# tkwa/iit

Measured on AMD Instinct MI355X. Metric: IIT (base,source) intervened pairs/sec, IOI GPT-2-small, IOI_ModelPair IIT+strict+behavior step, higher is better.
Workload: dtype bf16; 1 GPU; model=gpt2-small 12L/768d/12H (TL GPT-2 cfg, LNPre, gelu_new, V=50257), global_batch=256, seq_len=16, parallelism=dp1, engine=native, graphs=True

## Files before the change

csrc/gemm_dual.hip:

```cpp
#include "gemm_glds_body.h"

namespace {

template <int BM_, int BN_, int NS_, int NW_ = 4, int OCC_ = 2>
struct Cfg {
  static constexpr int BM = BM_, BN = BN_, NS = NS_, NW = NW_, OCC = OCC_;
  static constexpr int SMEM = GldsSmem<BM_, BN_, NS_, NW_, 64, OCC_>::BYTES;
};

struct Prefetch {
  const char* p[2];
  long bytes[2];
  int wgs;
};

__device__ __forceinline__ void prefetch_part(const Prefetch& pf, int part) {
  unsigned acc = 0u;
#pragma unroll
  for (int r = 0; r < 2; ++r) {
    if (!pf.p[r] || pf.bytes[r] <= 0) continue;
    const long gran = (pf.bytes[r] + 63) / 64;
    const long per = (gran + pf.wgs - 1) / pf.wgs;
    const long g0 = (long)part * per;
    const long g1 = g0 + per < gran ? g0 + per : gran;
    const char* base = pf.p[r];
    for (long g = g0 + threadIdx.x; g < g1; g += (long)blockDim.x * 8) {
      unsigned v[8];
#pragma unroll
      for (int u = 0; u < 8; ++u) {
        const long gg = g + (long)u * blockDim.x;
        v[u] = gg < g1 ? *(const unsigned*)(base + gg * 64) : 0u;
      }
#pragma unroll
      for (int u = 0; u < 8; ++u) acc ^= v[u];
    }
  }
  asm volatile("" ::"v"(acc));
}

template <class TW, int EW, class TX, int EX>
__global__ __launch_bounds__(TW::NW * 64, TW::OCC) void gemm_dual_kernel(G2Args pw, G2Args px, int w_tiles,
                                                                         int w_splits, int x_tiles, Prefetch pf) {
  static_assert(TW::NW == TX::NW && TW::OCC == TX::OCC, "one launch geometry");
  __shared__ __attribute__((aligned(16))) char smem[TW::SMEM > TX::SMEM ? TW::SMEM : TX::SMEM];
  if ((int)blockIdx.x < pf.wgs) {
    prefetch_part(pf, blockIdx.x);
    return;
  }
  const int b = blockIdx.x - pf.wgs;
  const int nw = w_tiles * w_splits;
  if (b < nw) {
    gemm_glds_body<TW::BM, TW::BN, TW::NS, true, true, EW, TW::NW, 64, TW::OCC>(pw, b % w_tiles, w_tiles,
                                                                                b / w_tiles, w_splits, smem);
// ... 135 lines not shown
```

csrc/layer_norm.hip:

```cpp
#include "common.h"
#include <initializer_list>
#include <stdlib.h>
#include <type_traits>

template <int W>
struct Pack;

template <>
struct Pack<4> {
  float4 v;
  static __device__ __forceinline__ Pack splat(float s) { return {make_float4(s, s, s, s)}; }
  static __device__ __forceinline__ Pack load(const float* p, long i) { return {((const float4*)p)[i]}; }
  static __device__ __forceinline__ Pack load(const __bf16* p, long i) {
    const bf16x4 t = ((const bf16x4*)p)[i];
    return {make_float4(bf2f(t[0]), bf2f(t[1]), bf2f(t[2]), bf2f(t[3]))};
  }
  template <class F, class... P>
  static __device__ __forceinline__ Pack map(F f, const P&... a) {
    return {make_float4(f(a.v.x...), f(a.v.y...), f(a.v.z...), f(a.v.w...))};
  }
  __device__ __forceinline__ float hsum() const { return (v.x + v.y) + (v.z + v.w); }
  template <int PIN>
  static __device__ __forceinline__ float dot(const Pack& a, const Pack& b) {
    if constexpr (PIN == 1)
// ... 41 lines not shown

struct RowSel {
  unsigned long long mask;
  int S;
  int Tb;
};

__device__ __forceinline__ bool sel_hit(const RowSel& sel, int row) {
  return sel.mask != 0ull && row < sel.Tb && ((sel.mask >> (row % sel.S)) & 1ull);
}

template <int W, int N>
__global__ __launch_bounds__(256) void ln_fwd_kernel(const float* __restrict__ x, const float* __restrict__ w,
                                                     const float* __restrict__ b, __bf16* __restrict__ y,
                                                     float* __restrict__ mean_out, float* __restrict__ rstd_out,
                                                     int T, int d, float eps, RowSel sel, float* __restrict__ y32) {
  using P = Pack<W>;
  const int row = blockIdx.x * 4 + (threadIdx.x >> 6);
  const int lane = threadIdx.x & 63;
  if (row >= T) return;
  const int dn = d / W;
  const long xat = (long)(sel_hit(sel, row) ? row + sel.Tb : row) * dn, yat = (long)row * dn;
  P v[N];
  float s = 0.f;
#pragma unroll
  for (int i = 0; i < N; ++i) {
    const int c = lane + i * 64;
    v[i] = c < dn ? P::load(x, xat + c) : P::splat(0.f);
    s += v[i].hsum();
  }
  const float mu = wave_sum(s) / d;
  float s2 = 0.f;
#pragma unroll
// ... 300 lines not shown
    if (n <= 1) f(W, ln_int<1>{}); else if (n <= 2) f(W, ln_int<2>{}); else if (n <= 3) f(W, ln_int<3>{});
    else if (n <= 4) f(W, ln_int<4>{}); else if (n <= 6) f(W, ln_int<6>{}); else if (n <= 8) f(W, ln_int<8>{});
    else if (n <= 12) f(W, ln_int<12>{}); else f(W, ln_int<16>{});
  } else {
    const ln_int<1> W;
    if (n <= 4) f(W, ln_int<4>{}); else if (n <= 16) f(W, ln_int<16>{}); else if (n <= 32) f(W, ln_int<32>{});
    else f(W, ln_int<64>{});
  }
}

template <class F>
static void ln_flag(bool b, F&& f) {
  if (b) f(std::true_type{}); else f(std::false_type{});
}

IIT_EXPORT int iit_ln_fwd(const float* x, const float* w, const float* b, void* y, float* y32, float* mean,
                          float* rstd, int T, int d, float eps, unsigned long long pos_mask, int S, int Tb,
                          void* stream) {
  if (pos_mask && (S <= 0 || S > 64 || 2 * (long)Tb > T)) return (int)hipErrorInvalidValue;
  const bool vec = ln_vec(d, {f32_rows(x), bf16_rows(y), f32_rows(y32), f32_rows(w), f32_rows(b)});
  if (d > 4096 || (y32 && !vec)) return (int)hipErrorInvalidValue;
  const RowSel sel{pos_mask, S > 0 ? S : 1, Tb};
  ln_dispatch(vec, d, [&](auto W, auto N) {
    hipLaunchKernelGGL((ln_fwd_kernel<W, N>), dim3((T + 3) / 4), dim3(256), 0, (hipStream_t)stream, x, w, b,
                       (__bf16*)y, mean, rstd, T, d, eps, sel, y32);
  });
  return hipGetLastError();
}

IIT_EXPORT int iit_ln_bwd_part_rows() { return 4 * ln_part_r(); }

IIT_EXPORT int iit_ln_bwd(const void* dy, int dy_f32, const void* x, int x_is_xhat16, const float* mean,
                          const float* rstd, const float* w, float* dx, const float* dres, void* dx16, float* dw,
                          float* db, float* part, const float* dy2, int T, int d, int accumulate,
                          unsigned long long pos_mask, int S, void* stream) {
  if (d > 4096 || (pos_mask && (S <= 0 || S > 64))) return (int)hipErrorInvalidValue;
  const LnPtr dyp = dy_f32 ? f32_rows(dy) : bf16_rows(dy), xp = x_is_xhat16 ? bf16_rows(x) : f32_rows(x);
  const bool vec = ln_vec(d, {dyp, xp, f32_rows(dx), f32_rows(dres), f32_rows(w), bf16_rows(dx16)});
  const bool fused = vec && !x_is_xhat16 && part && dw && db && d <= 1024 &&
                     ln_vec(d, {f32_rows(dw), f32_rows(db), f32_rows(part), f32_rows(dy2)});
  if ((dy2 && !fused) || (x_is_xhat16 && (!vec || w || dw || db))) return (int)hipErrorInvalidValue;
  const RowSel sel{pos_mask, S > 0 ? S : 1, T};
// ... 55 lines not shown
```

iit_amd/models/transformer.py:

```python
from __future__ import annotations

import math
import os
from typing import List, Optional, Union

import torch
from torch import nn

from ..engine.plan import RunPlan, Splice, scale_site as _scale_site, zero_grad_site as _zero_grad_site
from ..hooks.hook_points import HookedRootModule, HookPoint
from ..ops import select_ops
from ..ops.torch_ops import TorchOps
from .config import HookedTransformerConfig, make_config


def _hip_ops():
    from ..ops import hip_ops
    return hip_ops


def _flash_ok(q: torch.Tensor) -> bool:
    return q.is_cuda and q.dtype == torch.bfloat16 and _hip_ops().flash_supported(q)


# ... 70 lines not shown
        self.eps = cfg.eps
        self.rms = rms
        self.w = nn.Parameter(torch.ones(cfg.d_model)) if affine else None
        self.b = nn.Parameter(torch.zeros(cfg.d_model)) if (affine and not rms) else None
        self.hook_scale = HookPoint()
        self.hook_normalized = HookPoint()

    @staticmethod
    def make(cfg: HookedTransformerConfig, kind: Optional[str]) -> Optional["LayerNormSite"]:
        if kind is None:
            return None
        if kind not in ("LN", "LNPre", "RMS", "RMSPre"):
            raise NotImplementedError(f"normalization_type {kind}")
        return LayerNormSite(cfg, affine=kind in ("LN", "RMS"), rms=kind in ("RMS", "RMSPre"))

    def run(self, x, run: _Run, twin: bool = False):
        live = run.live(self.hook_scale) or run.live(self.hook_normalized)
        if self.rms:
            hs = (lambda t: run.site(self.hook_scale, t)) if live else None
            hn = (lambda t: run.site(self.hook_normalized, t)) if live else None
            return TorchOps.rms_norm(run.ops, x, self.w, self.eps, hook_scale=hs, hook_normalized=hn)
        if live or not run.ops.fused:
            return TorchOps.layer_norm(
                run.ops, x, self.w, self.b, self.eps,
                hook_scale=lambda t: run.site(self.hook_scale, t),
                hook_normalized=lambda t: run.site(self.hook_normalized, t),
            )
        if twin and self.w is not None and hasattr(run.ops, "layer_norm_twin"):
            return run.ops.layer_norm_twin(x, self.w, self.b, self.eps)
        return run.ops.layer_norm(x, self.w, self.b, self.eps)


def rotary_tables(cfg: HookedTransformerConfig):
    rd = cfg.rotary_dim or cfg.d_head
    pos = torch.arange(cfg.n_ctx, dtype=torch.float64)
    freq = cfg.rotary_base ** (-torch.arange(0, rd, 2, dtype=torch.float64) / rd)
    ang = pos[:, None] * freq[None, :]
    ang = ang.repeat_interleave(2, dim=-1) if cfg.rotary_adjacent_pairs else torch.cat([ang, ang], dim=-1)
    return ang.sin().float(), ang.cos().float()


class Attention(nn.Module):
    def __init__(self, cfg: HookedTransformerConfig, layer: int):
        super().__init__()
        H, d, dh = cfg.n_heads, cfg.d_model, cfg.d_head
# ... 149 lines not shown
        self.attn = Attention(cfg, layer)
        if not cfg.attn_only:
            self.mlp = MLP(cfg)
        self.hook_attn_in = HookPoint()
        self.hook_q_input = HookPoint()
        self.hook_k_input = HookPoint()
        self.hook_v_input = HookPoint()
        self.hook_mlp_in = HookPoint()
        self.hook_attn_out = HookPoint()
        self.hook_mlp_out = HookPoint()
        self.hook_resid_pre = HookPoint()
        if not cfg.attn_only:
            self.hook_resid_mid = HookPoint()
        self.hook_resid_post = HookPoint()

    def _norm(self, ln, x, run):
        if ln is None:
            return x.to(run.ops.dtype)
        return ln.run(x, run)

    def _norm_fork(self, ln, x, run):
        if ln is None or run.live(ln.hook_scale) or run.live(ln.hook_normalized) or not x.requires_grad:
            return self._norm(ln, x, run), x
        if ln.rms:
            fork = getattr(run.ops, "rms_norm_fork", None)
            out = fork(x, ln.w, ln.eps) if fork is not None else None
            return out if out is not None else (self._norm(ln, x, run), x)
        fork = getattr(run.ops, "layer_norm_fork", None)
        if fork is None:
            return self._norm(ln, x, run), x
        return fork(x, ln.w, ln.b, ln.eps)

    def last_position_ok(self, run: _Run) -> bool:
        if self.cfg.use_attn_result:
            return False
        sites = [self.hook_attn_out, self.hook_resid_post, self.hook_mlp_out]
        if not self.cfg.attn_only:
            sites += [self.hook_resid_mid, self.hook_mlp_in, self.mlp.hook_pre, self.mlp.hook_post]
            if self.mlp.gated:
                sites.append(self.mlp.hook_pre_linear)
            if self.ln2 is not None:
                sites += [self.ln2.hook_scale, self.ln2.hook_normalized]
        return not any(run.live(h) for h in sites)

    def forward(self, resid: torch.Tensor, run: _Run, last_only: bool = False) -> torch.Tensor:
        ops = run.ops
        attn = self.attn
        resid = run.site(self.hook_resid_pre, resid)

        spl = run.whole_splice(attn.hook_z.name)
        ln1_live = self.ln1 is not None and (run.live(self.ln1.hook_scale) or run.live(self.ln1.hook_normalized))
        if spl is not None and not attn.inner_live(run) and not ln1_live:
            z = run.site(attn.hook_z, spl.src.to(ops.dtype), spliced=True)
        else:
            x, resid = self._norm_fork(self.ln1, resid, run)
            z, spliced = attn.compute_z(x, run)
            z = run.site(attn.hook_z, z, spliced=spliced)
        if last_only:
            z, resid = z[:, -1:].contiguous(), resid[:, -1:].contiguous()
        attn_out_live = run.live(self.hook_attn_out) or self.cfg.use_attn_result
        if self.cfg.use_attn_result:
            result = run.site(attn.hook_result, ops.o_result(z, attn.W_O))
            attn_out = result.sum(-2) + ops.w(attn.b_O)
            attn_out = run.site(self.hook_attn_out, attn_out)
            resid_mid_pre = ops.residual(resid, attn_out)
        elif attn_out_live or not (ops.fused or getattr(ops, "fuses_residual", False)):
            attn_out = run.site(self.hook_attn_out, ops.o_proj(z, attn.W_O, attn.b_O))
            resid_mid_pre = ops.residual(resid, attn_out)
        else:
            resid_mid_pre = ops.o_proj_residual(z, attn.W_O, attn.b_O, resid)

        if self.cfg.attn_only:
            return run.site(self.hook_resid_post, resid_mid_pre)
        resid_mid = run.site(self.hook_resid_mid, resid_mid_pre)

        mlp = self.mlp
        spl = run.whole_splice(mlp.hook_post.name)
        ln2_live = self.ln2 is not None and (run.live(self.ln2.hook_scale) or run.live(self.ln2.hook_normalized))
        pre_lin_live = mlp.gated and run.live(mlp.hook_pre_linear)
        if spl is not None and not run.live(mlp.hook_pre) and not ln2_live and not pre_lin_live:
            post = run.site(mlp.hook_post, spl.src.to(ops.dtype), spliced=True)
        elif (not mlp.gated and getattr(ops, "mlp_gelu_residual", None) is not None
              and self.cfg.act_fn in ("gelu_new", "gelu_fast", "gelu_pytorch_tanh")
              and not (ln2_live or run.live(mlp.hook_pre) or run.live(mlp.hook_post) or run.live(self.hook_mlp_out))):
            x, resid_mid = self._norm_fork(self.ln2, resid_mid, run)
            resid_post = ops.mlp_gelu_residual(x, mlp.W_in, mlp.b_in, mlp.W_out, mlp.b_out, resid_mid)
            return run.site(self.hook_resid_post, resid_post)
        else:
            x, resid_mid = self._norm_fork(self.ln2, resid_mid, run)
            pre_hook = (lambda t: run.site(mlp.hook_pre, t)) if run.live(mlp.hook_pre) else None
            spliced = False
            if mlp.gated:
                lin_hook = (lambda t: run.site(mlp.hook_pre_linear, t)) if run.live(mlp.hook_pre_linear) else None
                pspl = run.plan.splice.get(mlp.hook_post.name) if run.plan is not None else None
                if pspl and len(pspl) == 1 and not pspl[0].whole and pre_hook is None and lin_hook is None:
                    _, post, spliced = TorchOps.mlp_gated_in(ops, x, mlp.W_gate, mlp.W_in, mlp.b_in,
                                                             self.cfg.act_fn, splice=pspl[0])
                else:
                    _, post = TorchOps.mlp_gated_in(ops, x, mlp.W_gate, mlp.W_in, mlp.b_in, self.cfg.act_fn,
                                                    hook_pre=pre_hook, hook_pre_linear=lin_hook)
            else:
                _, post = ops.mlp_in(x, mlp.W_in, mlp.b_in, self.cfg.act_fn, hook_pre=pre_hook)
            post = run.site(mlp.hook_post, post, spliced=spliced)
        if run.live(self.hook_mlp_out) or not (ops.fused or getattr(ops, "fuses_residual", False)):
# ... 10 lines not shown
            return False
        if self.ln1 is None or self.ln1.rms or (not cfg.attn_only and (self.ln2 is None or self.ln2.rms)):
            return False
        if not cfg.attn_only and (self.mlp.gated or cfg.act_fn not in ("gelu_new", "gelu_fast", "gelu_pytorch_tanh")):
            return False
        return True

    def forward_paired(self, p, run: _Run, sites, stop_after: str, captures, last_only: bool = False):
        ops = run.ops
        attn = self.attn
        zname = attn.hook_z.name
        zs = sites.get(zname)
        causal = self.cfg.attention_dir == "causal"
        S, H, dh = p.full.shape[1], self.cfg.n_heads, self.cfg.d_head
        mirror = ops.pair_heads_ok(S, dh) and H <= 64
        if zs is not None and any(ix.is_everything() for ix in zs):
            with torch.no_grad():
                x = ops.layer_norm(p.src, self.ln1.w, self.ln1.b, self.ln1.eps)
                q, k, v = ops.qkv(x, attn.W_Q, attn.W_K, attn.W_V, attn.b_Q, attn.b_K, attn.b_V)
                if mirror:
                    zf = ops.attention_dual(q, causal, attn.attn_scale)
                else:
                    z_src = ops.attention(q, k, v, causal, attn.attn_scale)
                    zf = torch.cat([z_src, z_src])
            z = _hip_ops().Paired(zf[:p.nb], zf)
            resid = p
        else:
            x, resid = ops.pair_layer_norm_fork(p, self.ln1.w, self.ln1.b, self.ln1.eps)
            qkv = ops.pair_qkv(x, attn.W_Q, attn.W_K, attn.W_V, attn.b_Q, attn.b_K, attn.b_V)
            heads, rest = None, list(zs or ())
            z = None
            if mirror and len(rest) == 1:
                heads = Splice(rest[0], None).head_mask(H)
                if heads is not None:
                    rest = []
                else:
                    z = ops.pair_attention_spliced(qkv, causal, attn.attn_scale, rest[0])
                    if z is not None:
                        rest = []
            if z is None:
                z = ops.pair_attention(qkv, causal, attn.attn_scale, heads=heads)
            for ix in rest:
                z = ops.pair_splice(z, ix)
        if zs is not None:
            captures[zname] = z.src
        if zname == stop_after:
            return self._finish_after_attn(z.base, resid.base, run, last_only), False
        resid_mid = ops.pair_o_proj_residual(z, attn.W_O, attn.b_O, resid)
        if self.cfg.attn_only:
            return resid_mid, True
        mlp = self.mlp
        pname = mlp.hook_post.name
        ps = sites.get(pname)
        erf = False
        if ps is None:
            x, resid2 = ops.pair_layer_norm_fork(resid_mid, self.ln2.w, self.ln2.b, self.ln2.eps)
            return ops.pair_mlp_gelu_residual(x, mlp.W_in, mlp.b_in, mlp.W_out, mlp.b_out, resid2, erf=erf), True
        if any(ix.is_everything() for ix in ps):
            with torch.no_grad():
                x = ops.layer_norm(resid_mid.src, self.ln2.w, self.ln2.b, self.ln2.eps)
                _, post_src = ops.mlp_in(x, mlp.W_in, mlp.b_in, self.cfg.act_fn)
            qf = torch.cat([post_src, post_src])
            post = _hip_ops().Paired(qf[:post_src.shape[0]], qf)
            resid2 = resid_mid
        else:
            x, resid2 = ops.pair_layer_norm_fork(resid_mid, self.ln2.w, self.ln2.b, self.ln2.eps)
            done = ops.pair_mlp_in(x, mlp.W_in, mlp.b_in, erf=erf, index=ps[0]) if len(ps) == 1 else None
            if done is not None:
                _, post = done
            else:
                _, post = ops.pair_mlp_in(x, mlp.W_in, mlp.b_in, erf=erf)
                for ix in ps:
                    post = ops.pair_splice(post, ix)
        captures[pname] = post.src
        if pname == stop_after:
            return ops.mlp_out_residual(post.base, mlp.W_out, mlp.b_out, resid2.base), False
        return ops.pair_mlp_out_residual(post, mlp.W_out, mlp.b_out, resid2), True

    def paired_torch_ok(self, ops) -> bool:
        cfg = self.cfg
        if getattr(ops, "fused", True) or ops.dtype != torch.bfloat16 or cfg.use_attn_result:
# ... 64 lines not shown
            return resid_mid
        mlp = self.mlp
        x = self.ln2.run(resid_mid, run)
        _, post = TorchOps.mlp_gated_in(ops, x, mlp.W_gate, mlp.W_in, mlp.b_in, self.cfg.act_fn)
        return ops.residual(resid_mid, ops.mlp_out(post, mlp.W_out, mlp.b_out))

    def _finish_after_attn(self, z, resid, run: _Run, last_only: bool):
        ops = run.ops
        attn = self.attn
        if last_only:
            z, resid = z[:, -1:].contiguous(), resid[:, -1:].contiguous()
        resid_mid = ops.o_proj_residual(z, attn.W_O, attn.b_O, resid)
        if self.cfg.attn_only:
            return resid_mid
        mlp = self.mlp
        x, resid_mid = self._norm_fork(self.ln2, resid_mid, run)
        return ops.mlp_gelu_residual(x, mlp.W_in, mlp.b_in, mlp.W_out, mlp.b_out, resid_mid)


def qkv_arena_groups(blocks, cfg):
    H, d, dh = cfg.n_heads, cfg.d_model, cfg.d_head
    groups = []
    for blk in blocks:
        a = blk.attn
        Hkv = a.n_kv
        Wq = a.W_Q
        Wk, Wv = (a._W_K, a._W_V) if a.gqa else (a.W_K, a.W_V)
        bq = a.b_Q
        bk, bv = (a._b_K, a._b_V) if a.gqa else (a.b_K, a.b_V)
        if Wq.shape != (H, d, dh) or Wk.shape != (Hkv, d, dh) or Wv.shape != (Hkv, d, dh):
            continue
# ... 346 lines not shown
```

iit_amd/ops/build.py:

```python
from __future__ import annotations

import hashlib
import os
import subprocess
import sys

ROOT = os.path.dirname(os.path.dirname(os.path.dirname(os.path.abspath(__file__))))
CSRC = os.path.join(ROOT, "csrc")
OUT_DIR = os.path.join(ROOT, "iit_amd", "_native")
LIB = os.path.join(OUT_DIR, "libiit_hip.so")
OBJ_CACHE = os.path.join(ROOT, "build", "objcache")
SOURCES = ["gemm.hip", "gemm_glds.hip", "gemm_edge.hip", "gemm_dual.hip", "gemm_8ph.hip", "gemm_4w.hip", "conv_nhwc.hip", "kernels.hip", "layer_norm.hip", "attn_mfma.hip", "flash_attn.hip", "llama_ops.hip",
           "splice.hip", "ioi_hl.hip", "bn_nhwc.hip", "gemm_f32.hip", "attn_fp32.hip"]
EXTRA_FLAGS = {"gemm_glds.hip": ["-mllvm", "-amdgpu-mfma-vgpr-form"], "gemm_edge.hip": ["-mllvm", "-amdgpu-mfma-vgpr-form"], "conv_nhwc.hip": ["-mllvm", "-amdgpu-mfma-vgpr-form"], "gemm_dual.hip": ["-mllvm", "-amdgpu-mfma-vgpr-form"],
               "gemm_8ph.hip": ["-mllvm", "-amdgpu-mfma-vgpr-form"]}
HEADERS = ["common.h", "gemm_glds_body.h", "gemm_w4.h", "splice_spec.h"]
ARCH = os.environ.get("IIT_OFFLOAD_ARCH", "gfx950")


def _hipcc() -> str:
    for c in (os.environ.get("HIPCC"), "/opt/rocm/bin/hipcc"):
        if c and os.path.exists(c):
            return c
    return "hipcc"


def sources():
    return [os.path.join(CSRC, s) for s in SOURCES if os.path.exists(os.path.join(CSRC, s))]


def source_hash() -> str:
# ... 63 lines not shown
```

iit_amd/ops/hip_kernels.py:

```python
from __future__ import annotations

import ctypes
import math
import os
from typing import Optional, Sequence

import numpy as np
import torch

from . import build as _build

c_void_p, c_long, c_int, c_float, c_ull = ctypes.c_void_p, ctypes.c_long, ctypes.c_int, ctypes.c_float, ctypes.c_ulonglong

EPI_BF16, EPI_BF16_BIAS3, EPI_F32_RESID, EPI_GELU, EPI_DGELU, EPI_F32_ACC, EPI_F32_ACC_QKV, EPI_F32_STORE = range(8)
EPI_GELU_ERF = 8
EPI_DGELU_ERF = 9
MODE_NN, MODE_AKM, MODE_BKM, MODE_AF32, MODE_BF32 = 0, 1, 2, 4, 8

_LIB = None
GEMM_GROUP_M = 4
GEMM_DUAL_GROUP_M = 2

_SIGS = {
    "iit_gemm": [c_void_p] * 10 + [c_long] * 5 + [c_int] * 12 + [c_void_p],
    "iit_gemm_f32": [c_void_p] * 6 + [c_long] * 4 + [c_int] * 7 + [c_void_p],
    "iit_gemm_f32_ok": [c_void_p] * 6 + [c_long] * 4 + [c_int] * 7,
    "iit_attn_f32_lds": [c_int] * 3,
    "iit_attn_f32_waves": [c_int] * 3,
    "iit_attn_f32_ok": [c_void_p] * 4 + [c_int] * 4,
    "iit_attn_f32_fwd": [c_void_p] * 6 + [c_int] * 4 + [c_float, c_int, c_void_p],
    "iit_attn_f32_bwd": [c_void_p] * 9 + [c_int] * 4 + [c_float, c_int, c_void_p],
    "iit_gemm_glds": [c_void_p] * 8 + [c_long] * 5 + [c_int] * 8 + [c_void_p] * 4,
    "iit_gemm_glds_ok": [c_void_p] * 5 + [c_long] * 5 + [c_int] * 9,
    "iit_gemm_glds_sm": [c_void_p] * 8 + [c_long] * 5 + [c_int] * 8 + [c_void_p] * 3 + [c_int] + [c_void_p] * 3,
    "iit_embed_pos_fwd": [c_void_p, c_void_p, c_void_p, c_void_p, c_int, c_int, c_int, c_void_p],
    "iit_embed_pos_bwd": [c_void_p, c_void_p, c_void_p, c_void_p, c_int, c_int, c_int, c_void_p],
    "iit_ln_fwd": [c_void_p] * 7 + [c_int, c_int, c_float, c_ull, c_int, c_int, c_void_p],
    "iit_ln_bwd": [c_void_p, c_int, c_void_p, c_int] + [c_void_p] * 10 + [c_int, c_int, c_int, c_ull, c_int, c_void_p],
    "iit_ln_bwd_part_rows": [],
    "iit_attn_small_fwd": [c_void_p] * 4 + [c_ull, c_int, c_int, c_int, c_int, c_long, c_long, c_long, c_float, c_int,
                                            c_void_p],
    "iit_attn_small_bwd": [c_void_p] * 4 + [c_ull, c_int, c_int, c_int, c_int, c_long, c_long, c_float, c_int, c_void_p],
    "iit_attn_mfma_fwd": [c_void_p] * 4 + [c_ull, c_int, c_int, c_int, c_int, c_long, c_long, c_long, c_float, c_int,
                                           c_void_p],
    "iit_attn_mfma_fwd_pair": [c_void_p] * 4 + [c_ull, c_int, c_int, c_int, c_int, c_long, c_long, c_long, c_float,
                                                c_int, c_void_p, c_int, c_ull, c_void_p],
    "iit_attn_mfma_bwd": [c_void_p] * 4 + [c_ull, c_int, c_int, c_int, c_int, c_long, c_long, c_float, c_int, c_void_p],
    "iit_attn_mfma_fwd_spec": [c_void_p] * 3 + [c_int] * 4 + [c_long, c_long, c_float, c_int, c_int, c_void_p,
                                                               c_void_p],
    "iit_attn_mfma_bwd_spec": [c_void_p] * 4 + [c_int] * 4 + [c_long, c_long, c_float, c_int, c_void_p, c_void_p],
    "iit_ce_fwd": [c_void_p, c_long, c_void_p, c_void_p, c_void_p, c_void_p, c_int, c_int, c_void_p],
    "iit_ce_bwd": [c_void_p, c_long, c_void_p, c_void_p, c_void_p, c_float, c_void_p, c_long, c_int, c_int, c_int,
# ... 466 lines not shown
def splice(act, src, out, n, spec_ptr, f32, mode, scale=1.0):
    if CHECK_BOUNDS:
        _bounds("iit_splice", ("act", act, 1, n, n), ("out", out, 1, n, n))
    _check(lib().iit_splice(_p(act), _p(src), _p(out), n, spec_ptr, int(f32), int(mode), float(scale), _stream()),
           "iit_splice")


def embed_pos_fwd(tokens, W_E, W_pos, out, B, S, d):
    _check(lib().iit_embed_pos_fwd(_p(tokens), _p(W_E), _p(W_pos), _p(out), B * S, S, d, _stream()), "embed_pos_fwd")


def embed_pos_bwd(tokens, g, dWE, dWpos, B, S, d):
    _check(lib().iit_embed_pos_bwd(_p(tokens), _p(g), _p(dWE), _p(dWpos), B, S, d, _stream()), "embed_pos_bwd")


def _ln_fwd(what, x, w, b, y, y32, mean, rstd, T, d, eps, pos_mask=0, S=1, Tb=0) -> int:
    if CHECK_BOUNDS:
        _bounds(what, ("x", x, T, d, d), ("y", y, T, d, d), ("y32", y32, T, d, d), ("mean", mean, 1, T, T),
                ("rstd", rstd, 1, T, T))
    return lib().iit_ln_fwd(_p(x), _p(w), _p(b), _p(y), _p(y32), _p(mean), _p(rstd), T, d, eps, pos_mask, S, Tb, _stream())


def ln_fwd(x, w, b, y, mean, rstd, T, d, eps):
    _check(_ln_fwd("ln_fwd", x, w, b, y, None, mean, rstd, T, d, eps), "ln_fwd")


def ln_fwd_twin(x, w, b, y, y32, mean, rstd, T, d, eps) -> bool:
    return _ln_fwd("ln_fwd_twin", x, w, b, y, y32, mean, rstd, T, d, eps) == 0


def ln_fwd_sel(x, w, b, y, mean, rstd, T, d, eps, pos_mask: int, S: int, Tb: int):
    _check(_ln_fwd("ln_fwd_sel", x, w, b, y, None, mean, rstd, T, d, eps, pos_mask, S, Tb), "ln_fwd_sel")


_LN_PART_ROWS = [0]


def _ln_part(dw, T: int, d: int):
    if dw is None or os.environ.get("IIT_LN_FUSED_DWDB", "1") == "0":
        return None
    rows = _LN_PART_ROWS[0] or lib().iit_ln_bwd_part_rows()
    _LN_PART_ROWS[0] = rows
    return torch.empty(((T + rows - 1) // rows) * 2 * d, dtype=torch.float32, device=dw.device)


def _ln_bwd(what, dy, x, mean, rstd, w, dx, dw, db, T, d, *, accumulate=False, dres=None, dx16=None, dy2=None,
            pos_mask=0, S=1, xh16=False):
# ... 518 lines not shown
```

iit_amd/ops/hip_ops.py:

```python
from __future__ import annotations

import math
import os
from typing import Optional, Sequence

import torch
from torch.autograd import Function

from ..engine import grad_hooks
from . import hip_kernels as K
from .gemm_dispatch import gemm, gemm_pair
from .torch_ops import TorchOps, act_fn

BF16 = torch.bfloat16
F32 = torch.float32


def _pad8(n: int) -> int:
    return (n + 7) // 8 * 8


def _grad_slot(p: Optional[torch.Tensor]) -> Optional[torch.Tensor]:
    if p is None or not p.requires_grad:
        return None
# ... 310 lines not shown
        ctx.params = (W_E, W_pos)
        return out

    @staticmethod
    def backward(ctx, g):
        if g is None:
            return None, None, None
        (tok,) = ctx.saved_tensors
        W_E, W_pos = ctx.params
        B, S = tok.shape
        K.embed_pos_bwd(tok, g.contiguous(), _grad_slot(W_E), _grad_slot(W_pos), B, S, W_E.shape[1])
        _done(W_E, W_pos)
        return None, None, None


def _xhat16(w, b, d: int) -> bool:
    return w is None and b is None and d % 4 == 0 and d <= 4096 and os.environ.get("IIT_LN_XHAT16", "1") == "1"


def _ln_forward(ctx, x, w, b, eps, x_full=None, twin=False, xhat16=False, pos_mask=0):
    ctx.set_materialize_grads(False)
    rows = x if x_full is None else x_full
    lead, d = rows.shape[:-1], rows.shape[-1]
    x2 = _flat2(rows.float().contiguous())
    T2 = x2.shape[0]
    T = T2 * x.shape[0] // rows.shape[0]
    S = x.shape[1] if x.dim() == 3 else 1
    if xhat16:
        yf = torch.empty(T2, d, dtype=BF16, device=x.device)
        y = yf.view(*lead, d)
    else:
        y = torch.empty(*lead, d, dtype=BF16, device=x.device)
        yf = y.view(T2, d)
    y32 = torch.empty(*lead, d, dtype=F32, device=x.device) if twin else None
    mean = torch.empty(T2, dtype=F32, device=x.device)
    rstd = torch.empty(T2, dtype=F32, device=x.device)
    if pos_mask:
        K.ln_fwd_sel(x2, w, b, yf, mean, rstd, T2, d, eps, pos_mask, S, T)
    elif not twin or not K.ln_fwd_twin(x2, w, b, yf, y32.view(T2, d), mean, rstd, T2, d, eps):
        K.ln_fwd(x2, w, b, yf, mean, rstd, T2, d, eps)
        if twin:
            y32.copy_(y)
    ctx.save_for_backward((yf if xhat16 else x2)[:T], mean[:T], rstd[:T])
    ctx.params = (w, b)
    ctx.in_dtype = x.dtype
    ctx.sel = (pos_mask, S)
    return y, y32


def _ln_backward(ctx, dy, dres=None, dy2=None, sel=None):
    if dy is None and dy2 is not None:
        dy, dy2 = dy2.float(), None
    if dy is None:
        return dres
    xs, mean, rstd = ctx.saved_tensors
# ... 964 lines not shown
    box = []
    out = fn.apply(*args, box)
    return out, box[0]


class HipOps(TorchOps):
    name = "hip"
    fused = True

    def __init__(self, model):
        super().__init__(BF16)
        self.model = model
        self.shadow = ModelShadow(model)
        pol = os.environ.get("IIT_DUAL_PREFETCH", "auto")
        self.prefetch = pol == "1" or (pol == "auto" and type(model).__name__ != "HookedEncoder")
        self._layer_of = {}
        for i, blk in enumerate(model.blocks):
            self._layer_of[id(blk.attn.W_Q)] = i
            self._layer_of[id(blk.attn.W_O)] = i
            if not model.cfg.attn_only:
                self._layer_of[id(blk.mlp.W_in)] = i
                self._layer_of[id(blk.mlp.W_out)] = i

    def begin_forward(self):
        self.shadow.ensure()
        _PF_SEQ.clear()
        _PF_ON[0] = self.prefetch

    def _L(self, p):
        return self.shadow.layers[self._layer_of[id(p)]]

    def embed(self, tokens, W_E):
        return W_E[tokens]

    def pos_embed(self, batch, seq, W_pos, offset: int = 0):
        return W_pos[offset:offset + seq].unsqueeze(0).expand(batch, seq, W_pos.shape[-1])

    def embed_pos(self, tokens, W_E, W_pos):
        return EmbedPosFn.apply(tokens, W_E, W_pos)

    def residual(self, a, b):
        return a.float() + b.float()

    def w(self, p: torch.Tensor) -> torch.Tensor:
        return p.to(BF16)

    def layer_norm(self, x, w, b, eps):
        return LayerNormFn.apply(x, w, b, eps)

    def layer_norm_twin(self, x, w, b, eps):
        if os.environ.get("IIT_LN_TWIN", "1") == "0":
            return LayerNormFn.apply(x, w, b, eps)
        y, y32 = LayerNormTwinFn.apply(x, w, b, eps)
        y._iit_f32 = (y.data_ptr(), y._version, y32)
        return y

    def layer_norm_fork(self, x, w, b, eps):
        return LayerNormForkFn.apply(x, w, b, eps)

    def qkv(self, x, W_Q, W_K, W_V, b_Q, b_K, b_V):
        i = self._layer_of[id(W_Q)]
        packed = QKVFn.apply(x, self.shadow.layers[i], self.shadow.biases[i], W_Q, W_K, W_V, b_Q, b_K, b_V)
        q, k, v = packed[:, :, 0], packed[:, :, 1], packed[:, :, 2]
        q._iit_packed = k._iit_packed = v._iit_packed = packed
        return q, k, v

    def attention(self, q, k, v, causal, attn_scale, patch_heads: Optional[Sequence[int]] = None, patch_src=None,
                  hook_scores=None, hook_pattern=None, ignore=float("-inf")):
        S, dh = q.shape[1], q.shape[-1]
        if S > 16 and flash_supported(q):
            packed = getattr(q, "_iit_packed", None)
            if packed is not None and getattr(k, "_iit_packed", None) is packed and \
                    getattr(v, "_iit_packed", None) is packed and packed.is_contiguous():
# ... 88 lines not shown
                best_v, best_i = v, i
            else:
                upd = v > best_v
                best_v = torch.where(upd, v, best_v)
                best_i = torch.where(upd, i, best_i)
        return best_i.view(*lead)


    supports_pairs = True

    def pair_embed_pos(self, tokens, src_tokens, W_E, W_pos) -> Paired:
        full_tok = torch.cat([tokens, src_tokens]).contiguous()
        out, full = _one(EmbedPosPairFn, tokens, W_E, W_pos, full_tok)
        return Paired(out, full)

    def pair_layer_norm_fork(self, p: Paired, w, b, eps):
        box = []
        y, x_pass = LayerNormForkPairFn.apply(p.base, w, b, eps, p.full.float().contiguous(), box)
        return Paired(y, box[0]), Paired(x_pass, p.full)

    def pair_layer_norm(self, p: Paired, w, b, eps, pos_mask: int = 0, twin: bool = False) -> Paired:
        box = []
        if twin and not pos_mask and w is not None and os.environ.get("IIT_LN_TWIN", "1") != "0":
            y, y32 = LayerNormPairTwinFn.apply(p.base, w, b, eps, p.full.float().contiguous(), box)
            yf, yf32 = box[0]
            y._iit_f32 = (y.data_ptr(), y._version, y32)
            return Paired(y, yf, (y32, yf32))
        y = LayerNormPairFn.apply(p.base, w, b, eps, p.full.float().contiguous(), box, int(pos_mask))
        return Paired(y, box[0])

    @staticmethod
    def position_mask(index, shape) -> int:
        if len(shape) != 3 or shape[1] > 64:
            return 0
        ranges = index.to_ranges(tuple(shape))
        if ranges is None or ranges[0] != [(0, shape[0])] or ranges[2] != [(0, shape[2])]:
            return 0
        m = 0
        for lo, hi in ranges[1]:
            for s_ in range(lo, hi):
                m |= 1 << s_
        return m

# ... 116 lines not shown
```

Measured before the change: 16830 pairs/s.

## Prefetch next-layer GEMM weights into L2 from extra layer-norm workgroups

Adds extra workgroups to the layer-norm forward kernel. They touch the bf16 weights of the following GEMMs (QKV/O, MLP in/out) so those weights are pulled into cache before the GEMM runs. The prefetch helper moves into a shared header and is threaded through the LN forward paths, including pair and fork variants, gated by IIT_FWD_PREFETCH (auto enables it for HookedTransformer). The aim is to hide weight-load latency in the small-batch GEMMs, at the cost of extra LN launch work and cache pressure.

```diff
diff --git a/csrc/gemm_dual.hip b/csrc/gemm_dual.hip
--- a/csrc/gemm_dual.hip
+++ b/csrc/gemm_dual.hip
@@ -1,4 +1,5 @@
 #include "gemm_glds_body.h"
+#include "prefetch.h"
 
 namespace {
 
@@ -8,35 +9,6 @@
   static constexpr int SMEM = GldsSmem<BM_, BN_, NS_, NW_, 64, OCC_>::BYTES;
 };
 
-struct Prefetch {
-  const char* p[2];
-  long bytes[2];
-  int wgs;
-};
-
-__device__ __forceinline__ void prefetch_part(const Prefetch& pf, int part) {
-  unsigned acc = 0u;
-#pragma unroll
-  for (int r = 0; r < 2; ++r) {
-    if (!pf.p[r] || pf.bytes[r] <= 0) continue;
-    const long gran = (pf.bytes[r] + 63) / 64;
-    const long per = (gran + pf.wgs - 1) / pf.wgs;
-    const long g0 = (long)part * per;
-    const long g1 = g0 + per < gran ? g0 + per : gran;
-    const char* base = pf.p[r];
-    for (long g = g0 + threadIdx.x; g < g1; g += (long)blockDim.x * 8) {
-      unsigned v[8];
-#pragma unroll
-      for (int u = 0; u < 8; ++u) {
-        const long gg = g + (long)u * blockDim.x;
-        v[u] = gg < g1 ? *(const unsigned*)(base + gg * 64) : 0u;
-      }
-#pragma unroll
-      for (int u = 0; u < 8; ++u) acc ^= v[u];
-    }
-  }
-  asm volatile("" ::"v"(acc));
-}
 
 template <class TW, int EW, class TX, int EX>
 __global__ __launch_bounds__(TW::NW * 64, TW::OCC) void gemm_dual_kernel(G2Args pw, G2Args px, int w_tiles,
diff --git a/csrc/layer_norm.hip b/csrc/layer_norm.hip
--- a/csrc/layer_norm.hip
+++ b/csrc/layer_norm.hip
@@ -1,4 +1,5 @@
 #include "common.h"
+#include "prefetch.h"
 #include <initializer_list>
 #include <stdlib.h>
 #include <type_traits>
@@ -79,9 +80,14 @@
 __global__ __launch_bounds__(256) void ln_fwd_kernel(const float* __restrict__ x, const float* __restrict__ w,
                                                      const float* __restrict__ b, __bf16* __restrict__ y,
                                                      float* __restrict__ mean_out, float* __restrict__ rstd_out,
-                                                     int T, int d, float eps, RowSel sel, float* __restrict__ y32) {
+                                                     int T, int d, float eps, RowSel sel, float* __restrict__ y32,
+                                                     Prefetch pf) {
   using P = Pack<W>;
-  const int row = blockIdx.x * 4 + (threadIdx.x >> 6);
+  if ((int)blockIdx.x < pf.wgs) {
+    prefetch_part(pf, blockIdx.x);
+    return;
+  }
+  const int row = (blockIdx.x - pf.wgs) * 4 + (threadIdx.x >> 6);
   const int lane = threadIdx.x & 63;
   if (row >= T) return;
   const int dn = d / W;
@@ -412,18 +418,28 @@
   if (b) f(std::true_type{}); else f(std::false_type{});
 }
 
-IIT_EXPORT int iit_ln_fwd(const float* x, const float* w, const float* b, void* y, float* y32, float* mean,
-                          float* rstd, int T, int d, float eps, unsigned long long pos_mask, int S, int Tb,
-                          void* stream) {
+IIT_EXPORT int iit_ln_fwd_pf(const float* x, const float* w, const float* b, void* y, float* y32, float* mean,
+                             float* rstd, int T, int d, float eps, unsigned long long pos_mask, int S, int Tb,
+                             const void* pf0, long pf0_bytes, const void* pf1, long pf1_bytes, int pf_wgs,
+                             void* stream) {
   if (pos_mask && (S <= 0 || S > 64 || 2 * (long)Tb > T)) return (int)hipErrorInvalidValue;
   const bool vec = ln_vec(d, {f32_rows(x), bf16_rows(y), f32_rows(y32), f32_rows(w), f32_rows(b)});
   if (d > 4096 || (y32 && !vec)) return (int)hipErrorInvalidValue;
   const RowSel sel{pos_mask, S > 0 ? S : 1, Tb};
+  Prefetch pf{{(const char*)pf0, (const char*)pf1}, {pf0 ? pf0_bytes & ~3L : 0, pf1 ? pf1_bytes & ~3L : 0}, 0};
+  if (((uintptr_t)pf0 | (uintptr_t)pf1) & 3) return (int)hipErrorInvalidValue;
+  if ((pf.bytes[0] > 0 || pf.bytes[1] > 0) && pf_wgs > 0) pf.wgs = pf_wgs < 1024 ? pf_wgs : 1024;
   ln_dispatch(vec, d, [&](auto W, auto N) {
-    hipLaunchKernelGGL((ln_fwd_kernel<W, N>), dim3((T + 3) / 4), dim3(256), 0, (hipStream_t)stream, x, w, b,
-                       (__bf16*)y, mean, rstd, T, d, eps, sel, y32);
+    hipLaunchKernelGGL((ln_fwd_kernel<W, N>), dim3(pf.wgs + (T + 3) / 4), dim3(256), 0, (hipStream_t)stream, x, w, b,
+                       (__bf16*)y, mean, rstd, T, d, eps, sel, y32, pf);
   });
   return hipGetLastError();
+}
+
+IIT_EXPORT int iit_ln_fwd(const float* x, const float* w, const float* b, void* y, float* y32, float* mean,
+                          float* rstd, int T, int d, float eps, unsigned long long pos_mask, int S, int Tb,
+                          void* stream) {
+  return iit_ln_fwd_pf(x, w, b, y, y32, mean, rstd, T, d, eps, pos_mask, S, Tb, nullptr, 0, nullptr, 0, 0, stream);
 }
 
 IIT_EXPORT int iit_ln_bwd_part_rows() { return 4 * ln_part_r(); }
diff --git a/csrc/prefetch.h b/csrc/prefetch.h
--- /dev/null
+++ b/csrc/prefetch.h
@@ -0,0 +1,31 @@
+#pragma once
+
+struct Prefetch {
+  const char* p[2];
+  long bytes[2];
+  int wgs;
+};
+
+__device__ __forceinline__ void prefetch_part(const Prefetch& pf, int part) {
+  unsigned acc = 0u;
+#pragma unroll
+  for (int r = 0; r < 2; ++r) {
+    if (!pf.p[r] || pf.bytes[r] <= 0) continue;
+    const long gran = (pf.bytes[r] + 63) / 64;
+    const long per = (gran + pf.wgs - 1) / pf.wgs;
+    const long g0 = (long)part * per;
+    const long g1 = g0 + per < gran ? g0 + per : gran;
+    const char* base = pf.p[r];
+    for (long g = g0 + threadIdx.x; g < g1; g += (long)blockDim.x * 8) {
+      unsigned v[8];
+#pragma unroll
+      for (int u = 0; u < 8; ++u) {
+        const long gg = g + (long)u * blockDim.x;
+        v[u] = gg < g1 ? *(const unsigned*)(base + gg * 64) : 0u;
+      }
+#pragma unroll
+      for (int u = 0; u < 8; ++u) acc ^= v[u];
+    }
+  }
+  asm volatile("" ::"v"(acc));
+}
diff --git a/iit_amd/models/transformer.py b/iit_amd/models/transformer.py
--- a/iit_amd/models/transformer.py
+++ b/iit_amd/models/transformer.py
@@ -108,7 +108,7 @@
             raise NotImplementedError(f"normalization_type {kind}")
         return LayerNormSite(cfg, affine=kind in ("LN", "RMS"), rms=kind in ("RMS", "RMSPre"))
 
-    def run(self, x, run: _Run, twin: bool = False):
+    def run(self, x, run: _Run, twin: bool = False, prefetch=None):
         live = run.live(self.hook_scale) or run.live(self.hook_normalized)
         if self.rms:
             hs = (lambda t: run.site(self.hook_scale, t)) if live else None
@@ -120,9 +120,10 @@
                 hook_scale=lambda t: run.site(self.hook_scale, t),
                 hook_normalized=lambda t: run.site(self.hook_normalized, t),
             )
+        kw = {} if prefetch is None else {"prefetch": prefetch}
         if twin and self.w is not None and hasattr(run.ops, "layer_norm_twin"):
-            return run.ops.layer_norm_twin(x, self.w, self.b, self.eps)
-        return run.ops.layer_norm(x, self.w, self.b, self.eps)
+            return run.ops.layer_norm_twin(x, self.w, self.b, self.eps, **kw)
+        return run.ops.layer_norm(x, self.w, self.b, self.eps, **kw)
 
 
 def rotary_tables(cfg: HookedTransformerConfig):
@@ -302,14 +303,19 @@
             self.hook_resid_mid = HookPoint()
         self.hook_resid_post = HookPoint()
 
-    def _norm(self, ln, x, run):
+    @staticmethod
+    def _fwd_prefetch(ops, *Ws):
+        f = getattr(ops, "fwd_prefetch", None)
+        return f(*Ws) if f is not None else None
+
+    def _norm(self, ln, x, run, prefetch=None):
         if ln is None:
             return x.to(run.ops.dtype)
-        return ln.run(x, run)
-
-    def _norm_fork(self, ln, x, run):
+        return ln.run(x, run, prefetch=prefetch)
+
+    def _norm_fork(self, ln, x, run, prefetch=None):
         if ln is None or run.live(ln.hook_scale) or run.live(ln.hook_normalized) or not x.requires_grad:
-            return self._norm(ln, x, run), x
+            return self._norm(ln, x, run, prefetch), x
         if ln.rms:
             fork = getattr(run.ops, "rms_norm_fork", None)
             out = fork(x, ln.w, ln.eps) if fork is not None else None
@@ -317,7 +323,7 @@
         fork = getattr(run.ops, "layer_norm_fork", None)
         if fork is None:
             return self._norm(ln, x, run), x
-        return fork(x, ln.w, ln.b, ln.eps)
+        return fork(x, ln.w, ln.b, ln.eps, **({} if prefetch is None else {"prefetch": prefetch}))
 
     def last_position_ok(self, run: _Run) -> bool:
         if self.cfg.use_attn_result:
@@ -341,7 +347,7 @@
         if spl is not None and not attn.inner_live(run) and not ln1_live:
             z = run.site(attn.hook_z, spl.src.to(ops.dtype), spliced=True)
         else:
-            x, resid = self._norm_fork(self.ln1, resid, run)
+            x, resid = self._norm_fork(self.ln1, resid, run, self._fwd_prefetch(ops, attn.W_Q, attn.W_O))
             z, spliced = attn.compute_z(x, run)
             z = run.site(attn.hook_z, z, spliced=spliced)
         if last_only:
@@ -371,11 +377,11 @@
         elif (not mlp.gated and getattr(ops, "mlp_gelu_residual", None) is not None
               and self.cfg.act_fn in ("gelu_new", "gelu_fast", "gelu_pytorch_tanh")
               and not (ln2_live or run.live(mlp.hook_pre) or run.live(mlp.hook_post) or run.live(self.hook_mlp_out))):
-            x, resid_mid = self._norm_fork(self.ln2, resid_mid, run)
+            x, resid_mid = self._norm_fork(self.ln2, resid_mid, run, self._fwd_prefetch(ops, mlp.W_in, mlp.W_out))
             resid_post = ops.mlp_gelu_residual(x, mlp.W_in, mlp.b_in, mlp.W_out, mlp.b_out, resid_mid)
             return run.site(self.hook_resid_post, resid_post)
         else:
-            x, resid_mid = self._norm_fork(self.ln2, resid_mid, run)
+            x, resid_mid = self._norm_fork(self.ln2, resid_mid, run, self._fwd_prefetch(ops, mlp.W_in, mlp.W_out))
             pre_hook = (lambda t: run.site(mlp.hook_pre, t)) if run.live(mlp.hook_pre) else None
             spliced = False
             if mlp.gated:
@@ -416,9 +422,10 @@
         causal = self.cfg.attention_dir == "causal"
         S, H, dh = p.full.shape[1], self.cfg.n_heads, self.cfg.d_head
         mirror = ops.pair_heads_ok(S, dh) and H <= 64
+        pf1 = ops.fwd_prefetch(attn.W_Q, attn.W_O)
         if zs is not None and any(ix.is_everything() for ix in zs):
             with torch.no_grad():
-                x = ops.layer_norm(p.src, self.ln1.w, self.ln1.b, self.ln1.eps)
+                x = ops.layer_norm(p.src, self.ln1.w, self.ln1.b, self.ln1.eps, prefetch=pf1)
                 q, k, v = ops.qkv(x, attn.W_Q, attn.W_K, attn.W_V, attn.b_Q, attn.b_K, attn.b_V)
                 if mirror:
                     zf = ops.attention_dual(q, causal, attn.attn_scale)
@@ -428,7 +435,7 @@
             z = _hip_ops().Paired(zf[:p.nb], zf)
             resid = p
         else:
-            x, resid = ops.pair_layer_norm_fork(p, self.ln1.w, self.ln1.b, self.ln1.eps)
+            x, resid = ops.pair_layer_norm_fork(p, self.ln1.w, self.ln1.b, self.ln1.eps, prefetch=pf1)
             qkv = ops.pair_qkv(x, attn.W_Q, attn.W_K, attn.W_V, attn.b_Q, attn.b_K, attn.b_V)
             heads, rest = None, list(zs or ())
             z = None
@@ -455,18 +462,19 @@
         pname = mlp.hook_post.name
         ps = sites.get(pname)
         erf = False
+        pf2 = ops.fwd_prefetch(mlp.W_in, mlp.W_out)
         if ps is None:
-            x, resid2 = ops.pair_layer_norm_fork(resid_mid, self.ln2.w, self.ln2.b, self.ln2.eps)
+            x, resid2 = ops.pair_layer_norm_fork(resid_mid, self.ln2.w, self.ln2.b, self.ln2.eps, prefetch=pf2)
             return ops.pair_mlp_gelu_residual(x, mlp.W_in, mlp.b_in, mlp.W_out, mlp.b_out, resid2, erf=erf), True
         if any(ix.is_everything() for ix in ps):
             with torch.no_grad():
-                x = ops.layer_norm(resid_mid.src, self.ln2.w, self.ln2.b, self.ln2.eps)
+                x = ops.layer_norm(resid_mid.src, self.ln2.w, self.ln2.b, self.ln2.eps, prefetch=pf2)
                 _, post_src = ops.mlp_in(x, mlp.W_in, mlp.b_in, self.cfg.act_fn)
             qf = torch.cat([post_src, post_src])
             post = _hip_ops().Paired(qf[:post_src.shape[0]], qf)
             resid2 = resid_mid
         else:
-            x, resid2 = ops.pair_layer_norm_fork(resid_mid, self.ln2.w, self.ln2.b, self.ln2.eps)
+            x, resid2 = ops.pair_layer_norm_fork(resid_mid, self.ln2.w, self.ln2.b, self.ln2.eps, prefetch=pf2)
             done = ops.pair_mlp_in(x, mlp.W_in, mlp.b_in, erf=erf, index=ps[0]) if len(ps) == 1 else None
             if done is not None:
                 _, post = done
@@ -561,7 +569,7 @@
         if self.cfg.attn_only:
             return resid_mid
         mlp = self.mlp
-        x, resid_mid = self._norm_fork(self.ln2, resid_mid, run)
+        x, resid_mid = self._norm_fork(self.ln2, resid_mid, run, self._fwd_prefetch(ops, mlp.W_in, mlp.W_out))
         return ops.mlp_gelu_residual(x, mlp.W_in, mlp.b_in, mlp.W_out, mlp.b_out, resid_mid)
 
 
diff --git a/iit_amd/ops/build.py b/iit_amd/ops/build.py
--- a/iit_amd/ops/build.py
+++ b/iit_amd/ops/build.py
@@ -14,7 +14,7 @@
            "splice.hip", "ioi_hl.hip", "bn_nhwc.hip", "gemm_f32.hip", "attn_fp32.hip"]
 EXTRA_FLAGS = {"gemm_glds.hip": ["-mllvm", "-amdgpu-mfma-vgpr-form"], "gemm_edge.hip": ["-mllvm", "-amdgpu-mfma-vgpr-form"], "conv_nhwc.hip": ["-mllvm", "-amdgpu-mfma-vgpr-form"], "gemm_dual.hip": ["-mllvm", "-amdgpu-mfma-vgpr-form"],
                "gemm_8ph.hip": ["-mllvm", "-amdgpu-mfma-vgpr-form"]}
-HEADERS = ["common.h", "gemm_glds_body.h", "gemm_w4.h", "splice_spec.h"]
+HEADERS = ["common.h", "gemm_glds_body.h", "gemm_w4.h", "splice_spec.h", "prefetch.h"]
 ARCH = os.environ.get("IIT_OFFLOAD_ARCH", "gfx950")
 
 
diff --git a/iit_amd/ops/hip_kernels.py b/iit_amd/ops/hip_kernels.py
--- a/iit_amd/ops/hip_kernels.py
+++ b/iit_amd/ops/hip_kernels.py
@@ -36,6 +36,8 @@
     "iit_embed_pos_fwd": [c_void_p, c_void_p, c_void_p, c_void_p, c_int, c_int, c_int, c_void_p],
     "iit_embed_pos_bwd": [c_void_p, c_void_p, c_void_p, c_void_p, c_int, c_int, c_int, c_void_p],
     "iit_ln_fwd": [c_void_p] * 7 + [c_int, c_int, c_float, c_ull, c_int, c_int, c_void_p],
+    "iit_ln_fwd_pf": [c_void_p] * 7 + [c_int, c_int, c_float, c_ull, c_int, c_int, c_void_p, c_long, c_void_p, c_long,
+                      c_int, c_void_p],
     "iit_ln_bwd": [c_void_p, c_int, c_void_p, c_int] + [c_void_p] * 10 + [c_int, c_int, c_int, c_ull, c_int, c_void_p],
     "iit_ln_bwd_part_rows": [],
     "iit_attn_small_fwd": [c_void_p] * 4 + [c_ull, c_int, c_int, c_int, c_int, c_long, c_long, c_long, c_float, c_int,
@@ -532,23 +534,47 @@
     _check(lib().iit_embed_pos_bwd(_p(tokens), _p(g), _p(dWE), _p(dWpos), B, S, d, _stream()), "embed_pos_bwd")
 
 
-def _ln_fwd(what, x, w, b, y, y32, mean, rstd, T, d, eps, pos_mask=0, S=1, Tb=0) -> int:
+def prefetch_wgs(nbytes: int, per_mb: float) -> int:
+    gran = int(nbytes) // 64
+    if gran <= 0 or per_mb <= 0:
+        return 0
+    return max(1, min(1024, gran, int(nbytes / 2 ** 20 * per_mb)))
+
+
+def _ln_prefetch_args(prefetch, wgs):
+    ts = [t for t in (prefetch or ()) if t is not None and t.is_cuda and t.is_contiguous()][:2]
+    nb = [t.numel() * t.element_size() // 64 * 64 for t in ts]
+    if wgs is None:
+        wgs = prefetch_wgs(sum(nb), _PF_PER_MB)
+    if not any(nb) or wgs <= 0:
+        return (None, 0, None, 0, 0)
+    ts += [None] * (2 - len(ts))
+    nb += [0] * (2 - len(nb))
+    return (_p(ts[0]), nb[0], _p(ts[1]), nb[1], int(wgs))
+
+
+def _ln_fwd(what, x, w, b, y, y32, mean, rstd, T, d, eps, pos_mask=0, S=1, Tb=0, prefetch=None,
+            pf_wgs=None) -> int:
     if CHECK_BOUNDS:
         _bounds(what, ("x", x, T, d, d), ("y", y, T, d, d), ("y32", y32, T, d, d), ("mean", mean, 1, T, T),
                 ("rstd", rstd, 1, T, T))
-    return lib().iit_ln_fwd(_p(x), _p(w), _p(b), _p(y), _p(y32), _p(mean), _p(rstd), T, d, eps, pos_mask, S, Tb, _stream())
-
-
-def ln_fwd(x, w, b, y, mean, rstd, T, d, eps):
-    _check(_ln_fwd("ln_fwd", x, w, b, y, None, mean, rstd, T, d, eps), "ln_fwd")
-
-
-def ln_fwd_twin(x, w, b, y, y32, mean, rstd, T, d, eps) -> bool:
-    return _ln_fwd("ln_fwd_twin", x, w, b, y, y32, mean, rstd, T, d, eps) == 0
-
-
-def ln_fwd_sel(x, w, b, y, mean, rstd, T, d, eps, pos_mask: int, S: int, Tb: int):
-    _check(_ln_fwd("ln_fwd_sel", x, w, b, y, None, mean, rstd, T, d, eps, pos_mask, S, Tb), "ln_fwd_sel")
+    return lib().iit_ln_fwd_pf(_p(x), _p(w), _p(b), _p(y), _p(y32), _p(mean), _p(rstd), T, d, eps, pos_mask, S, Tb,
+                               *_ln_prefetch_args(prefetch, pf_wgs), _stream())
+
+
+def ln_fwd(x, w, b, y, mean, rstd, T, d, eps, prefetch=None, pf_wgs=None):
+    _check(_ln_fwd("ln_fwd", x, w, b, y, None, mean, rstd, T, d, eps, prefetch=prefetch, pf_wgs=pf_wgs),
+           "ln_fwd")
+
+
+def ln_fwd_twin(x, w, b, y, y32, mean, rstd, T, d, eps, prefetch=None, pf_wgs=None) -> bool:
+    return _ln_fwd("ln_fwd_twin", x, w, b, y, y32, mean, rstd, T, d, eps, prefetch=prefetch,
+                   pf_wgs=pf_wgs) == 0
+
+
+def ln_fwd_sel(x, w, b, y, mean, rstd, T, d, eps, pos_mask: int, S: int, Tb: int, prefetch=None, pf_wgs=None):
+    _check(_ln_fwd("ln_fwd_sel", x, w, b, y, None, mean, rstd, T, d, eps, pos_mask, S, Tb, prefetch=prefetch,
+                   pf_wgs=pf_wgs), "ln_fwd_sel")
 
 
 _LN_PART_ROWS = [0]
diff --git a/iit_amd/ops/hip_ops.py b/iit_amd/ops/hip_ops.py
--- a/iit_amd/ops/hip_ops.py
+++ b/iit_amd/ops/hip_ops.py
@@ -348,12 +348,24 @@
         return None, None, None
 
 
+_LN_PF: list = [None]
+
+
+def _ln_apply(fn, prefetch, *args):
+    _LN_PF[0] = prefetch
+    try:
+        return fn.apply(*args)
+    finally:
+        _LN_PF[0] = None
+
+
 def _xhat16(w, b, d: int) -> bool:
     return w is None and b is None and d % 4 == 0 and d <= 4096 and os.environ.get("IIT_LN_XHAT16", "1") == "1"
 
 
 def _ln_forward(ctx, x, w, b, eps, x_full=None, twin=False, xhat16=False, pos_mask=0):
     ctx.set_materialize_grads(False)
+    prefetch = _LN_PF[0]
     rows = x if x_full is None else x_full
     lead, d = rows.shape[:-1], rows.shape[-1]
     x2 = _flat2(rows.float().contiguous())
@@ -370,9 +382,9 @@
     mean = torch.empty(T2, dtype=F32, device=x.device)
     rstd = torch.empty(T2, dtype=F32, device=x.device)
     if pos_mask:
-        K.ln_fwd_sel(x2, w, b, yf, mean, rstd, T2, d, eps, pos_mask, S, T)
-    elif not twin or not K.ln_fwd_twin(x2, w, b, yf, y32.view(T2, d), mean, rstd, T2, d, eps):
-        K.ln_fwd(x2, w, b, yf, mean, rstd, T2, d, eps)
+        K.ln_fwd_sel(x2, w, b, yf, mean, rstd, T2, d, eps, pos_mask, S, T, prefetch=prefetch)
+    elif not twin or not K.ln_fwd_twin(x2, w, b, yf, y32.view(T2, d), mean, rstd, T2, d, eps, prefetch=prefetch):
+        K.ln_fwd(x2, w, b, yf, mean, rstd, T2, d, eps, prefetch=prefetch)
         if twin:
             y32.copy_(y)
     ctx.save_for_backward((yf if xhat16 else x2)[:T], mean[:T], rstd[:T])
@@ -1367,18 +1379,23 @@
         self.shadow = ModelShadow(model)
         pol = os.environ.get("IIT_DUAL_PREFETCH", "auto")
         self.prefetch = pol == "1" or (pol == "auto" and type(model).__name__ != "HookedEncoder")
+        self.fwd_pf = False
         self._layer_of = {}
+        self._mirror_key = {}
         for i, blk in enumerate(model.blocks):
-            self._layer_of[id(blk.attn.W_Q)] = i
-            self._layer_of[id(blk.attn.W_O)] = i
+            mats = [(blk.attn.W_Q, "qkv"), (blk.attn.W_O, "o")]
             if not model.cfg.attn_only:
-                self._layer_of[id(blk.mlp.W_in)] = i
-                self._layer_of[id(blk.mlp.W_out)] = i
+                mats += [(blk.mlp.W_in, "in"), (blk.mlp.W_out, "out")]
+            for W, key in mats:
+                self._layer_of[id(W)] = i
+                self._mirror_key[id(W)] = key
 
     def begin_forward(self):
         self.shadow.ensure()
         _PF_SEQ.clear()
         _PF_ON[0] = self.prefetch
+        pol = os.environ.get("IIT_FWD_PREFETCH", "auto")
+        self.fwd_pf = pol == "1" or (pol == "auto" and type(self.model).__name__ == "HookedTransformer")
 
     def _L(self, p):
         return self.shadow.layers[self._layer_of[id(p)]]
@@ -1398,18 +1415,23 @@
     def w(self, p: torch.Tensor) -> torch.Tensor:
         return p.to(BF16)
 
-    def layer_norm(self, x, w, b, eps):
-        return LayerNormFn.apply(x, w, b, eps)
-
-    def layer_norm_twin(self, x, w, b, eps):
+    def fwd_prefetch(self, *Ws):
+        if not self.fwd_pf:
+            return None
+        return tuple(self._L(W)[self._mirror_key[id(W)]] for W in Ws)
+
+    def layer_norm(self, x, w, b, eps, prefetch=None):
+        return _ln_apply(LayerNormFn, prefetch, x, w, b, eps)
+
+    def layer_norm_twin(self, x, w, b, eps, prefetch=None):
         if os.environ.get("IIT_LN_TWIN", "1") == "0":
-            return LayerNormFn.apply(x, w, b, eps)
-        y, y32 = LayerNormTwinFn.apply(x, w, b, eps)
+            return _ln_apply(LayerNormFn, prefetch, x, w, b, eps)
+        y, y32 = _ln_apply(LayerNormTwinFn, prefetch, x, w, b, eps)
         y._iit_f32 = (y.data_ptr(), y._version, y32)
         return y
 
-    def layer_norm_fork(self, x, w, b, eps):
-        return LayerNormForkFn.apply(x, w, b, eps)
+    def layer_norm_fork(self, x, w, b, eps, prefetch=None):
+        return _ln_apply(LayerNormForkFn, prefetch, x, w, b, eps)
 
     def qkv(self, x, W_Q, W_K, W_V, b_Q, b_K, b_V):
         i = self._layer_of[id(W_Q)]
@@ -1528,19 +1550,19 @@
         out, full = _one(EmbedPosPairFn, tokens, W_E, W_pos, full_tok)
         return Paired(out, full)
 
-    def pair_layer_norm_fork(self, p: Paired, w, b, eps):
+    def pair_layer_norm_fork(self, p: Paired, w, b, eps, prefetch=None):
         box = []
-        y, x_pass = LayerNormForkPairFn.apply(p.base, w, b, eps, p.full.float().contiguous(), box)
+        y, x_pass = _ln_apply(LayerNormForkPairFn, prefetch, p.base, w, b, eps, p.full.float().contiguous(), box)
         return Paired(y, box[0]), Paired(x_pass, p.full)
 
-    def pair_layer_norm(self, p: Paired, w, b, eps, pos_mask: int = 0, twin: bool = False) -> Paired:
+    def pair_layer_norm(self, p: Paired, w, b, eps, pos_mask: int = 0, twin: bool = False, prefetch=None) -> Paired:
         box = []
         if twin and not pos_mask and w is not None and os.environ.get("IIT_LN_TWIN", "1") != "0":
-            y, y32 = LayerNormPairTwinFn.apply(p.base, w, b, eps, p.full.float().contiguous(), box)
+            y, y32 = _ln_apply(LayerNormPairTwinFn, prefetch, p.base, w, b, eps, p.full.float().contiguous(), box)
             yf, yf32 = box[0]
             y._iit_f32 = (y.data_ptr(), y._version, y32)
             return Paired(y, yf, (y32, yf32))
-        y = LayerNormPairFn.apply(p.base, w, b, eps, p.full.float().contiguous(), box, int(pos_mask))
+        y = _ln_apply(LayerNormPairFn, prefetch, p.base, w, b, eps, p.full.float().contiguous(), box, int(pos_mask))
         return Paired(y, box[0])
 
     @staticmethod
```

Result: faster. 17070 pairs/s, median of 6 (+1.4%).
